# sm-edwards/CrossScale-ECG-A-Modular-HPC-Pipeline-from-Locality-Optimization-to-MPI-GPU-Overlap

Hardware: AMD Instinct MI355X
Metric: ECG samples/sec (node) + conv1d speedup vs torch.Conv1d, tiny 1D-CNN at 1/2/4/8 GPU (higher is better)
Workload: dtype bf16; 1 GPU; model=TinyECG (1458 params), global_batch=256, seq_len=500, parallelism=dp1, sync=fedavg every 50 local steps (none all_reduce AVG, overlap=none), per_client_batch=256, max_windows_per_client=20000, backend=fused

## Files before the change

csrc/kernels/tiny_ecg_step.hip:

```cpp
#include "../include/ecg_common.h"

#include <climits>
#include <cstdint>
#include <cstdlib>
#include <cstring>
#include <type_traits>

namespace {

constexpr int C = 16;
constexpr int K1 = 7;
constexpr int K2 = 5;
constexpr int MAX_CLASSES = 16;
constexpr int MAX_PAIRS_PER_WAVE = 4;

struct Layout {
  int w1, b1, w2, b2, wh, bh, P;
};

__host__ __device__ inline Layout make_layout(int nc) {
  Layout l;
  l.w1 = 0;
  l.b1 = C * K1;
  l.w2 = l.b1 + C;
  l.b2 = l.w2 + C * C * K2;
  l.wh = l.b2 + C;
  l.bh = l.wh + nc * C;
  l.P = l.bh + nc;
  return l;
}

struct Smem {
  int Lp;
  int xs_off, xcol_off, h1_off, dh2_off, ps_off, frag_off, red_off, bytes;
};

constexpr int RED_G = 0;
constexpr int RED_POOLED = 16;
constexpr int RED_POOL = 48;

struct FusedOpt {
  int slab_wt;
};
__host__ __device__ constexpr int msplit(int waves) { return (waves - 1) / 5 < 1 ? 1 : (waves - 1) / 5; }
__host__ __device__ constexpr int red_cnt(int waves) { return RED_POOL + waves * 16; }
__host__ __device__ constexpr int red_m(int waves) { return red_cnt(waves) + waves * 16; }
__host__ __device__ constexpr int red_dw1(int waves) { return red_m(waves) + msplit(waves) * 1280; }
__host__ __device__ constexpr int red_head(int waves) { return red_dw1(waves) + waves * 128; }
__host__ __device__ constexpr int red_floats(int waves) { return red_head(waves) + 288; }

__device__ __forceinline__ __amdgpu_buffer_rsrc_t make_rsrc(const void* p, long bytes) {
  return __builtin_amdgcn_make_buffer_rsrc(const_cast<void*>(p), (short)0, (int)bytes, 0x00020000);
}
__device__ __forceinline__ void st_wt(__amdgpu_buffer_rsrc_t r, int idx, float v) {
  __builtin_amdgcn_raw_buffer_store_b32(__builtin_bit_cast(unsigned, v), r, idx * 4, 0, 16);
}
__device__ __forceinline__ void st_wt4(__amdgpu_buffer_rsrc_t r, int idx, f32x4 v) {
  typedef int i32x4 __attribute__((ext_vector_type(4)));
  __builtin_amdgcn_raw_buffer_store_b128(__builtin_bit_cast(i32x4, v), r, idx * 4, 0, 16);
}
__device__ __forceinline__ float ld_wt(__amdgpu_buffer_rsrc_t r, int idx) {
  return __builtin_bit_cast(float, __builtin_amdgcn_raw_buffer_load_b32(r, idx * 4, 0, 16));
}

constexpr int F32_KSTEPS = C * K2 / 4;

constexpr int WP_FRAGF = 0;
constexpr int WP_FRAGD = 3 * 64 * 8;
constexpr int WP_AW1 = 2 * 3 * 64 * 8;
constexpr int WP_B2_BYTE = (WP_AW1 + C * 8) * 2;
constexpr int WP_BYTES = WP_B2_BYTE + C * 4;
constexpr int kParamsW2End = C * K1 + C + C * C * K2;

__host__ __device__ constexpr int frag_bias_elem(int co) { return (2 * 64 + 32 + co) * 8; }
__host__ __device__ constexpr bool frag_pad_is_bias(int which, int l, int j) { return which == 0 && j == 0 && l < 48; }

__device__ __forceinline__ void wprep_put(unsigned char* wp, int i, float v) {
  __bf16* wb = reinterpret_cast<__bf16*>(wp);
  if (i < C * K1) {
    wb[WP_AW1 + (i / K1) * 8 + i % K1] = ecg::to_bf16(v);
  } else if (i < C * K1 + C) {
    wb[WP_AW1 + (i - C * K1) * 8 + 7] = ecg::to_bf16(v);
  } else if (i < kParamsW2End) {
    const int e = i - (C * K1 + C);
    const int co = e / (C * K2), ci = (e / K2) % C, k = e % K2;
    const int rf = 16 * k + ci, rd = 16 * k + co;
    const __bf16 bv = ecg::to_bf16(v);
    wb[WP_FRAGF + ((rf >> 5) * 64 + 16 * ((rf & 31) >> 3) + co) * 8 + (rf & 7)] = bv;
    wb[WP_FRAGD + ((rd >> 5) * 64 + 16 * ((rd & 31) >> 3) + ci) * 8 + (rd & 7)] = bv;
  } else if (i < kParamsW2End + C) {
    reinterpret_cast<float*>(wp + WP_B2_BYTE)[i - kParamsW2End] = v;
    wb[WP_FRAGF + frag_bias_elem(i - kParamsW2End)] = ecg::to_bf16(v);
  }
}

__global__ __launch_bounds__(256) void tiny_prep_kernel(const float* __restrict__ params,
                                                        unsigned char* __restrict__ wp,
                                                        const int* __restrict__ idx_src, int* __restrict__ idx_dst,
                                                        long n_idx) {
  const int tid = threadIdx.x;
  if (blockIdx.x == 0) {
    for (int i = tid; i < kParamsW2End + C; i += 256) wprep_put(wp, i, params[i]);
    __bf16* wb = reinterpret_cast<__bf16*>(wp);
    for (int e = tid; e < 2 * 32 * 8; e += 256) {
      const int which = e >> 8, l = 32 + ((e >> 3) & 31), j = e & 7;
      if (!frag_pad_is_bias(which, l, j)) wb[(which ? WP_FRAGD : WP_FRAGF) + (2 * 64 + l) * 8 + j] = ecg::to_bf16(0.f);
    }
    return;
  }
  const long base = (long)(blockIdx.x - 1) * 1024;
  for (long i = base + tid; i < n_idx && i < base + 1024; i += 256) idx_dst[i] = idx_src[i];
}

__host__ __device__ inline Smem make_smem(int L, int waves, int nc = MAX_CLASSES, bool f32 = false) {
  Smem s;
  s.Lp = (L + 31) / 32 * 32;
  s.xs_off = 0;
  s.xcol_off = s.xs_off + ((s.Lp + 16) * 4 + 15) / 16 * 16;
  s.h1_off = s.xcol_off + (f32 ? 0 : (s.Lp + 1) * 16);
  const int act_bytes = (s.Lp + 8) * C * (f32 ? 4 : 2);
  s.dh2_off = s.h1_off + act_bytes;
  s.ps_off = s.dh2_off + act_bytes;
  const int ps_bytes = ((make_layout(nc).P) * 4 + 15) / 16 * 16;
  s.frag_off = s.ps_off + ps_bytes;
  s.red_off = s.frag_off + (f32 ? 2 * F32_KSTEPS * 64 * 4 : 2 * 3 * 64 * 16);
  s.bytes = s.red_off + (red_floats(waves) * 4 + 15) / 16 * 16;
  return s;
}

__device__ __forceinline__ bf16x8 cat44(s16x4 a, s16x4 b) {
  typedef short s16x8 __attribute__((ext_vector_type(8)));
  s16x8 r;
  r[0] = a[0]; r[1] = a[1]; r[2] = a[2]; r[3] = a[3];
  r[4] = b[0]; r[5] = b[1]; r[6] = b[2]; r[7] = b[3];
  return __builtin_bit_cast(bf16x8, r);
}

__device__ __forceinline__ s16x4 lds_tr16(const __bf16* p) {
  return __builtin_amdgcn_ds_read_tr16_b64_v4i16((__attribute__((address_space(3))) s16x4*)(p));
}

__device__ __forceinline__ float lane_bcast(float v, int src) {
  return __builtin_bit_cast(float, __builtin_amdgcn_readlane(__builtin_bit_cast(int, v), src));
}

__device__ __forceinline__ float row16_sum(float v) {
  v += __builtin_bit_cast(float, __builtin_amdgcn_update_dpp(0, __builtin_bit_cast(int, v), 0x111, 0xf, 0xf, true));
  v += __builtin_bit_cast(float, __builtin_amdgcn_update_dpp(0, __builtin_bit_cast(int, v), 0x112, 0xf, 0xf, true));
  v += __builtin_bit_cast(float, __builtin_amdgcn_update_dpp(0, __builtin_bit_cast(int, v), 0x114, 0xf, 0xf, true));
  v += __builtin_bit_cast(float, __builtin_amdgcn_update_dpp(0, __builtin_bit_cast(int, v), 0x118, 0xf, 0xf, true));
  return v;
}

template <int WAVES, bool F32, bool PF = false>
struct TinySample {
  static_assert(!(PF && F32), "prepared fragments are bf16 operands");
  using AT = std::conditional_t<F32, float, __bf16>;
  static constexpr int NT = WAVES * 64;
  Smem sm;
  Layout lay;
  int L, Lp, NP, nc;
  int tid, lane, w, h, c;
  float* xs;
  __bf16* xcol;
  AT* h1s;
  AT* ms;
  float* ps;
  __bf16* fragF;
  __bf16* fragD;
  float* fragF32;
  float* fragD32;
  float* red;
  uint32_t mask1 = 0u;
  bf16x8 pf_aw, pf_wf[3], pf_wd[3];

  __device__ __forceinline__ void pf_load_fwd(const unsigned char* __restrict__ wp) {
    const __bf16* wb = reinterpret_cast<const __bf16*>(wp);
    if (h == 0) {
      pf_aw = *reinterpret_cast<const bf16x8*>(wb + WP_AW1 + c * 8);
    } else {
#pragma unroll
      for (int j = 0; j < 8; ++j) pf_aw[j] = ecg::to_bf16(0.f);
    }
#pragma unroll
    for (int s = 0; s < 3; ++s) pf_wf[s] = *reinterpret_cast<const bf16x8*>(wb + WP_FRAGF + (s * 64 + lane) * 8);
  }
  __device__ __forceinline__ void pf_load_dgrad(const unsigned char* __restrict__ wp) {
    const __bf16* wb = reinterpret_cast<const __bf16*>(wp);
    if (w == 0) {
#pragma unroll
      for (int s = 0; s < 3; ++s) pf_wd[s] = *reinterpret_cast<const bf16x8*>(wb + WP_FRAGD + (s * 64 + lane) * 8);
    }
  }

  __device__ __forceinline__ TinySample(unsigned char* smem, int L_, int nc_)
      : sm(make_smem(L_, WAVES, nc_, F32)), lay(make_layout(nc_)), L(L_), nc(nc_) {
    Lp = sm.Lp;
    NP = Lp / 32;
    xs = reinterpret_cast<float*>(smem + sm.xs_off);
    xcol = reinterpret_cast<__bf16*>(smem + sm.xcol_off);
    h1s = reinterpret_cast<AT*>(smem + sm.h1_off);
    ms = reinterpret_cast<AT*>(smem + sm.dh2_off);
    ps = reinterpret_cast<float*>(smem + sm.ps_off);
    fragF = reinterpret_cast<__bf16*>(smem + sm.frag_off);
    fragD = fragF + 3 * 64 * 8;
    fragF32 = reinterpret_cast<float*>(smem + sm.frag_off);
    fragD32 = fragF32 + F32_KSTEPS * 64;
    red = reinterpret_cast<float*>(smem + sm.red_off);
    tid = threadIdx.x;
    lane = tid & 63;
    w = __builtin_amdgcn_readfirstlane(tid >> 6);
    h = lane >> 4;
    c = lane & 15;
  }

  static constexpr int XK = (32 * MAX_PAIRS_PER_WAVE * WAVES + 16 + NT - 1) / NT;
  struct XRegs {
    float v[XK];
  };
  __device__ __forceinline__ void load_x(const float* __restrict__ xrow, XRegs& r) const {
#pragma unroll
    for (int k = 0; k < XK; ++k) {
      const int i = tid + k * NT, t = i - 3;
      if (k * NT < Lp + 16) {
        const float v = xrow[min(max(t, 0), L - 1)];
        r.v[k] = (i < Lp + 16 && t >= 0 && t < L) ? v : 0.f;
      }
    }
  }
  __device__ __forceinline__ void put_x(const XRegs& r) {
#pragma unroll
    for (int k = 0; k < XK; ++k) {
      const int i = tid + k * NT;
      if (i < Lp + 16) xs[i] = r.v[k];
    }
  }
  __device__ __forceinline__ void stage_x(const float* __restrict__ xrow) {
    XRegs r;
    load_x(xrow, r);
    put_x(r);
  }

  __device__ __forceinline__ void put_param(int i, float v) {
    ps[i] = v;
    if constexpr (!F32) {
      if (i >= lay.b2 && i < lay.b2 + C) fragF[frag_bias_elem(i - lay.b2)] = ecg::to_bf16(v);
    }
    const int e = i - lay.w2;
    if (e >= 0 && e < C * C * K2) {
      const int co = e / (C * K2), ci = (e / K2) % C, k = e % K2;
      const int rf = 16 * k + ci, rd = 16 * k + co;
      if constexpr (F32) {
        fragF32[(rf >> 2) * 64 + 16 * (rf & 3) + co] = v;
        fragD32[(rd >> 2) * 64 + 16 * (rd & 3) + ci] = v;
      } else {
        const __bf16 bv = ecg::to_bf16(v);
        fragF[((rf >> 5) * 64 + 16 * ((rf & 31) >> 3) + co) * 8 + (rf & 7)] = bv;
        fragD[((rd >> 5) * 64 + 16 * ((rd & 31) >> 3) + ci) * 8 + (rd & 7)] = bv;
      }
    }
  }

  __device__ __forceinline__ void zero_pads() {
    if constexpr (!F32) {
      for (int e = PF ? 2 * 32 * 8 : tid; e < 2 * 32 * 8; e += NT) {
        const int which = e >> 8, l = 32 + ((e >> 3) & 31), j = e & 7;
        if (!frag_pad_is_bias(which, l, j)) (which ? fragD : fragF)[(2 * 64 + l) * 8 + j] = ecg::to_bf16(0.f);
      }
      if (tid < 4) reinterpret_cast<uint32_t*>(xcol + Lp * 8)[tid] = 0u;
    }
    constexpr int DW = C * (int)sizeof(AT) / 4;
    uint32_t* h1w = reinterpret_cast<uint32_t*>(h1s);
    uint32_t* mw = reinterpret_cast<uint32_t*>(ms);
    for (int i = tid; i < 8 * DW; i += NT) {
      const int r = i / DW, d = i % DW;
      const int hr = r < 2 ? r : Lp + 2 + (r - 2);
      h1w[hr * DW + d] = 0u;
      const int dr = r < 4 ? r : Lp + 4 + (r - 4);
      mw[dr * DW + d] = 0u;
    }
  }

  __device__ __forceinline__ void conv1() {
    if constexpr (!F32) {
      bf16x8 Aw;
      if constexpr (PF) {
        Aw = pf_aw;
      } else {
#pragma unroll
        for (int j = 0; j < 8; ++j) {
          const float v = j < K1 ? ps[lay.w1 + c * K1 + j] : ps[lay.b1 + c];
          Aw[j] = ecg::to_bf16(h == 0 ? v : 0.f);
        }
      }
      const __bf16* xb = xcol + (h == 0 ? (lane & 15) * 8 : Lp * 8);
      const int tstride = h == 0 ? 16 * 8 : 0;
      const int ntiles = Lp / 16;
      const int j0 = 2 * h;
#pragma unroll 1
      for (int pi = 0; pi < 2 * MAX_PAIRS_PER_WAVE; pi += 2) {
        if (w + pi * WAVES >= ntiles) break;
        int tile[2];
        float v0[2], v1[2];
#pragma unroll
        for (int u = 0; u < 2; ++u) {
          tile[u] = min(w + (pi + u) * WAVES, ntiles - 1);
          const int t = 16 * tile[u] + (lane & 15);
          v0[u] = xs[t + j0];
          v1[u] = j0 + 1 < K1 ? xs[t + j0 + 1] : 1.f;
        }
        const bool has2 = w + (pi + 1) * WAVES < ntiles;
#pragma unroll
        for (int u = 0; u < 2; ++u) {
          const int t = 16 * tile[u] + (lane & 15);
          const bool tv = t < L;
          bf16x2 pr;
          pr[0] = ecg::to_bf16(tv ? v0[u] : 0.f);
          pr[1] = ecg::to_bf16(tv ? v1[u] : 0.f);
          *reinterpret_cast<bf16x2*>(xcol + t * 8 + j0) = pr;
        }
        bf16x8 Bx[2];
#pragma unroll
        for (int u = 0; u < 2; ++u) Bx[u] = *reinterpret_cast<const bf16x8*>(xb + tile[u] * tstride);
#pragma unroll
        for (int u = 0; u < 2; ++u) {
          if (u == 1 && !has2) break;
          const f32x4 acc = __builtin_amdgcn_mfma_f32_16x16x32_bf16(Aw, Bx[u], f32x4{0.f, 0.f, 0.f, 0.f}, 0, 0, 0);
          bf16x4 o;
#pragma unroll
          for (int i = 0; i < 4; ++i) o[i] = (AT)fmaxf(acc[i], 0.f);
          *reinterpret_cast<bf16x4*>(h1s + (16 * tile[u] + (lane & 15) + 2) * C + 4 * h) = o;
        }
      }
      return;
    }
    mask1 = 0u;
    float w1r[K1];
#pragma unroll
    for (int k = 0; k < K1; ++k) w1r[k] = ps[lay.w1 + c * K1 + k];
    const float b1r = ps[lay.b1 + c];
#pragma unroll
    for (int pi = 0; pi < MAX_PAIRS_PER_WAVE; ++pi) {
      const int pair = w + pi * WAVES;
      if (pair < NP) {
#pragma unroll
        for (int half = 0; half < 2; ++half) {
          const int t0 = 32 * pair + 16 * half + 4 * h;
          float xw[12];
#pragma unroll
          for (int q4 = 0; q4 < 3; ++q4) {
            const float4 v = reinterpret_cast<const float4*>(xs + t0)[q4];
            xw[4 * q4] = v.x; xw[4 * q4 + 1] = v.y; xw[4 * q4 + 2] = v.z; xw[4 * q4 + 3] = v.w;
          }
#pragma unroll
          for (int i = 0; i < 4; ++i) {
            const int t = t0 + i;
            float v = b1r;
#pragma unroll
            for (int k = 0; k < K1; ++k) v = fmaf(w1r[k], xw[i + k], v);
            v = (t < L) ? fmaxf(v, 0.f) : 0.f;
            const AT vb = (AT)v;
            h1s[(t + 2) * C + c] = vb;
            mask1 |= ((float)vb > 0.f ? 1u : 0u) << (pi * 8 + half * 4 + i);
          }
        }
      }
    }
  }

  __device__ __forceinline__ void conv2() {
    if constexpr (!F32) {
      bf16x8 Wf[3];
      float pool[4];
      if constexpr (PF) {
#pragma unroll
        for (int s = 0; s < 3; ++s) Wf[s] = pf_wf[s];
      } else {
#pragma unroll
        for (int s = 0; s < 3; ++s) Wf[s] = *reinterpret_cast<const bf16x8*>(fragF + (s * 64 + lane) * 8);
      }
      bf16x8 Bone;
#pragma unroll
      for (int j = 0; j < 8; ++j) Bone[j] = ecg::to_bf16(0.f);
      if (h == 2) Bone[0] = ecg::to_bf16(1.f);
#pragma unroll
      for (int i = 0; i < 4; ++i) pool[i] = 0.f;
#pragma unroll
      for (int pi = 0; pi < MAX_PAIRS_PER_WAVE; ++pi) {
        const int pair = w + pi * WAVES;
        if (pair < NP) {
          bf16x8 Bh[2][3];
#pragma unroll
          for (int half = 0; half < 2; ++half)
#pragma unroll
            for (int s = 0; s < 3; ++s) {
              const int r = 32 * pair + 16 * half + (lane & 15) + 2 * s + (h >> 1) - 2;
              if (s == 2 && h >= 2)
                Bh[half][s] = Bone;
              else
                Bh[half][s] = *reinterpret_cast<const bf16x8*>(h1s + (r + 2) * C + 8 * (h & 1));
            }
          f32x4 accs[2];
#pragma unroll
          for (int half = 0; half < 2; ++half) {
            accs[half] = f32x4{0.f, 0.f, 0.f, 0.f};
#pragma unroll
            for (int s = 0; s < 3; ++s)
              accs[half] = __builtin_amdgcn_mfma_f32_16x16x32_bf16(Wf[s], Bh[half][s], accs[half], 0, 0, 0);
          }
          auto epilogue = [&](auto masked) {
#pragma unroll
            for (int half = 0; half < 2; ++half) {
              const int t = 32 * pair + 16 * half + (lane & 15);
              const bool tv = !decltype(masked)::value || t < L;
              bf16x4 mk;
#pragma unroll
              for (int i = 0; i < 4; ++i) {
                const float a = tv ? accs[half][i] : 0.f;
                pool[i] += fmaxf(a, 0.f);
                mk[i] = ecg::to_bf16(__builtin_amdgcn_fmed3f(a * 0x1p126f, 0.f, 1.f));
              }
              *reinterpret_cast<bf16x4*>(ms + (t + 4) * C + 4 * h) = mk;
            }
          };
          if (32 * pair + 32 <= L)
            epilogue(std::false_type{});
          else
            epilogue(std::true_type{});
        }
      }
#pragma unroll
      for (int i = 0; i < 4; ++i) pool[i] = row16_sum(pool[i]);
      if ((lane & 15) == 15) {
#pragma unroll
        for (int i = 0; i < 4; ++i) red[RED_POOL + w * 16 + 4 * h + i] = pool[i];
      }
      return;
    }
    bf16x8 Bf[3];
    float Wf[F32_KSTEPS];
    if constexpr (F32) {
#pragma unroll
      for (int s = 0; s < F32_KSTEPS; ++s) Wf[s] = fragF32[s * 64 + lane];
    } else {
#pragma unroll
      for (int s = 0; s < 3; ++s) Bf[s] = *reinterpret_cast<const bf16x8*>(fragF + (s * 64 + lane) * 8);
    }
    const float b2r = ps[lay.b2 + c];
    float pool = 0.f, cnt = 0.f;
#pragma unroll
    for (int pi = 0; pi < MAX_PAIRS_PER_WAVE; ++pi) {
      const int pair = w + pi * WAVES;
      if (pair < NP) {
#pragma unroll
        for (int half = 0; half < 2; ++half) {
          const int t0 = 32 * pair + 16 * half;
          f32x4 acc = {0.f, 0.f, 0.f, 0.f};
          if constexpr (F32) {
#pragma unroll
            for (int s = 0; s < F32_KSTEPS; ++s) {
              const int r = 4 * s + h, tap = r >> 4, ci = r & 15;
              const float a = h1s[(t0 + (lane & 15) + tap - 2 + 2) * C + ci];
              acc = __builtin_amdgcn_mfma_f32_16x16x4f32(a, Wf[s], acc, 0, 0, 0);
            }
          } else {
#pragma unroll
            for (int s = 0; s < 3; ++s) {
              const int tap = 2 * s + (h >> 1);
              const int r = t0 + (lane & 15) + tap - 2;
              const bf16x8 A = *reinterpret_cast<const bf16x8*>(h1s + (r + 2) * C + 8 * (h & 1));
              acc = __builtin_amdgcn_mfma_f32_16x16x32_bf16(A, Bf[s], acc, 0, 0, 0);
            }
          }
#pragma unroll
          for (int i = 0; i < 4; ++i) {
            const int t = t0 + 4 * h + i;
            float v = fmaxf(acc[i] + b2r, 0.f);
            if (t >= L) v = 0.f;
            pool += v;
            const bool on = v > 0.f;
            cnt += on ? 1.f : 0.f;
            ms[(t + 4) * C + c] = (AT)(on ? 1.f : 0.f);
          }
        }
      }
    }
    pool = ecg::quarter_sum(pool);
    cnt = ecg::quarter_sum(cnt);
    if (lane < 16) {
      red[RED_POOL + w * 16 + lane] = pool;
      red[red_cnt(WAVES) + w * 16 + lane] = cnt;
    }
  }

  template <bool TRAIN>
  __device__ __forceinline__ void head_and_M(int ylab, float inv_B, float* out, int out_stride, int b) {
    if (w == 0) {
      float pp[WAVES];
#pragma unroll
      for (int ww = 0; ww < WAVES; ++ww) pp[ww] = red[RED_POOL + ww * 16 + c];
      float pooled = 0.f;
#pragma unroll
      for (int ww = 0; ww < WAVES; ++ww) pooled += pp[ww];
      pooled *= 1.0f / (float)L;
      float pv[C];
#pragma unroll
      for (int co = 0; co < C; ++co) pv[co] = lane_bcast(pooled, co);
      const int n = c;
      float logit = -INFINITY;
      if (n < nc) {
        const float4* whr = reinterpret_cast<const float4*>(ps + lay.wh + n * C);
        logit = ps[lay.bh + n];
#pragma unroll
        for (int q4 = 0; q4 < C / 4; ++q4) {
          const float4 wv4 = whr[q4];
          logit = fmaf(wv4.x, pv[4 * q4], logit);
          logit = fmaf(wv4.y, pv[4 * q4 + 1], logit);
          logit = fmaf(wv4.z, pv[4 * q4 + 2], logit);
          logit = fmaf(wv4.w, pv[4 * q4 + 3], logit);
        }
      }
      if constexpr (!TRAIN) {
        if (lane < nc) out[(long)b * out_stride + n] = logit;
      } else {
        float m = -INFINITY;
        for (int nn = 0; nn < nc; ++nn) m = fmaxf(m, lane_bcast(logit, nn));
        const float e = (n < nc) ? __expf(logit - m) : 0.f;
        float ssum = 0.f;
        for (int nn = 0; nn < nc; ++nn) ssum += lane_bcast(e, nn);
        const int y = __builtin_amdgcn_readfirstlane(ylab);
        const float loss = m + __logf(ssum) - lane_bcast(logit, y);
        const float dlogit = (n < nc) ? (e / ssum - (n == y ? 1.f : 0.f)) * inv_B : 0.f;
        float* hg = red + red_head(WAVES);
        if (lane < nc) {
          float4* hr = reinterpret_cast<float4*>(hg + n * C);
#pragma unroll
          for (int q4 = 0; q4 < C / 4; ++q4)
            hr[q4] = make_float4(dlogit * pv[4 * q4], dlogit * pv[4 * q4 + 1], dlogit * pv[4 * q4 + 2],
                                 dlogit * pv[4 * q4 + 3]);
          hg[nc * C + n] = dlogit;
        }
        if (lane == 0) hg[nc * C + nc] = loss;
        float dp = 0.f;
        for (int nn = 0; nn < nc; ++nn) dp = fmaf(lane_bcast(dlogit, nn), ps[lay.wh + nn * C + c], dp);
        const float gl = dp * (1.0f / (float)L);
        if (lane < 16) red[RED_G + c] = gl;
        if constexpr (PF) {
          float gq[8];
#pragma unroll
          for (int j = 0; j < 8; ++j) {
            const float lo = lane_bcast(gl, j), hi = lane_bcast(gl, 8 + j);
            gq[j] = (h & 1) ? hi : lo;
          }
#pragma unroll
          for (int s = 0; s < 3; ++s) {
            bf16x8 sc;
#pragma unroll
            for (int j = 0; j < 8; ++j) sc[j] = ecg::to_bf16(ecg::from_bf16(pf_wd[s][j]) * gq[j]);
            *reinterpret_cast<bf16x8*>(fragD + (s * 64 + lane) * 8) = sc;
          }
        }
      }
    } else if (TRAIN && w <= 5 * msplit(WAVES)) {
      constexpr int S = msplit(WAVES);
      const int item = w - 1, k = item / S, part = item % S;
      const int per = (NP + S - 1) / S;
      const int p0 = part * per, p1 = p0 + per < NP ? p0 + per : NP;
      f32x4 acc = {0.f, 0.f, 0.f, 0.f};
      if constexpr (F32) {
        for (int pair = p0; pair < p1; ++pair) {
#pragma unroll
          for (int s = 0; s < 8; ++s) {
            const int t = 32 * pair + 4 * s + h;
            const float a = ms[(t + 4) * C + (lane & 15)];
            const float bb = h1s[(t + k - 2 + 2) * C + (lane & 15)];
            acc = __builtin_amdgcn_mfma_f32_16x16x4f32(a, bb, acc, 0, 0, 0);
          }
        }
      } else {
        const int q = (lane & 15) >> 2, p4 = (lane & 3) * 4;
        bf16x8 ones;
#pragma unroll
        for (int j = 0; j < 8; ++j) ones[j] = ecg::to_bf16(1.f);
        f32x4 cnt1 = {0.f, 0.f, 0.f, 0.f}, cnt2 = {0.f, 0.f, 0.f, 0.f};
        auto mfma_pair = [&](int pair, f32x4 a, f32x4& cn) {
          const int ta = 32 * pair + 4 * h + q;
          const bf16x8 A = cat44(lds_tr16(ms + (ta + 4) * C + p4), lds_tr16(ms + (ta + 16 + 4) * C + p4));
          const bf16x8 Bm =
              cat44(lds_tr16(h1s + (ta + k - 2 + 2) * C + p4), lds_tr16(h1s + (ta + 16 + k - 2 + 2) * C + p4));
          if (k == 2) cn = __builtin_amdgcn_mfma_f32_16x16x32_bf16(A, ones, cn, 0, 0, 0);
          return __builtin_amdgcn_mfma_f32_16x16x32_bf16(A, Bm, a, 0, 0, 0);
        };
        f32x4 acc2 = {0.f, 0.f, 0.f, 0.f};
        int pair = p0;
        for (; pair + 1 < p1; pair += 2) {
          acc = mfma_pair(pair, acc, cnt1);
          acc2 = mfma_pair(pair + 1, acc2, cnt2);
        }
        if (pair < p1) acc = mfma_pair(pair, acc, cnt1);
#pragma unroll
        for (int i = 0; i < 4; ++i) acc[i] += acc2[i];
        if (k == 2 && (lane & 15) == 0) {
#pragma unroll
          for (int i = 0; i < 4; ++i) red[red_cnt(WAVES) + part * 16 + 4 * h + i] = cnt1[i] + cnt2[i];
        }
      }
      float* pm = red + red_m(WAVES) + part * 1280;
#pragma unroll
      for (int i = 0; i < 4; ++i) pm[(4 * h + i) * (C * K2) + c * K2 + k] = acc[i];
    }
  }

  __device__ __forceinline__ void dgrad() {
    float gq[8];
#pragma unroll
    for (int q2 = 0; q2 < 2; ++q2) {
      const float4 v = reinterpret_cast<const float4*>(red + RED_G + 8 * (h & 1))[q2];
      gq[4 * q2] = v.x; gq[4 * q2 + 1] = v.y; gq[4 * q2 + 2] = v.z; gq[4 * q2 + 3] = v.w;
    }
    bf16x8 Bd[3];
    float Wd[F32_KSTEPS];
    if constexpr (!F32) {
      if constexpr (PF) {
#pragma unroll
        for (int s = 0; s < 3; ++s) Bd[s] = *reinterpret_cast<const bf16x8*>(fragD + (s * 64 + lane) * 8);
      } else {
#pragma unroll
        for (int s = 0; s < 3; ++s) {
          const bf16x8 raw = *reinterpret_cast<const bf16x8*>(fragD + (s * 64 + lane) * 8);
#pragma unroll
          for (int j = 0; j < 8; ++j) Bd[s][j] = ecg::to_bf16(ecg::from_bf16(raw[j]) * gq[j]);
        }
      }
      const int q = (lane & 15) >> 2, p4 = (lane & 3) * 4;
      const __bf16* xzero = xcol + Lp * 8;
      f32x4 wacc = {0.f, 0.f, 0.f, 0.f};
#pragma unroll
      for (int pi = 0; pi < MAX_PAIRS_PER_WAVE; ++pi) {
        const int pair = w + pi * WAVES;
        if (pair < NP) {
          bf16x8 Am[2][3];
          bf16x4 hv[2];
          const __bf16* mbase = ms + (32 * pair + (lane & 15) - (h >> 1) + 2) * C + 8 * (h & 1);
#pragma unroll
          for (int half = 0; half < 2; ++half) {
            const int t0 = 32 * pair + 16 * half;
#pragma unroll
            for (int s = 0; s < 3; ++s)
              Am[half][s] = *reinterpret_cast<const bf16x8*>(mbase + (16 * half + 4 - 2 * s) * C);
            hv[half] = *reinterpret_cast<const bf16x4*>(h1s + (t0 + (lane & 15) + 2) * C + 4 * h);
          }
          f32x4 accs[2];
#pragma unroll
          for (int half = 0; half < 2; ++half) {
            accs[half] = f32x4{0.f, 0.f, 0.f, 0.f};
#pragma unroll
            for (int s = 0; s < 3; ++s)
              accs[half] = __builtin_amdgcn_mfma_f32_16x16x32_bf16(Bd[s], Am[half][s], accs[half], 0, 0, 0);
          }
#pragma unroll
          for (int half = 0; half < 2; ++half) {
            const int t0 = 32 * pair + 16 * half;
            typedef unsigned u32x2 __attribute__((ext_vector_type(2)));
            const u32x2 hb = __builtin_bit_cast(u32x2, hv[half]);
            u32x2 db;
#pragma unroll
            for (int q2 = 0; q2 < 2; ++q2) {
              const unsigned nz = (hb[q2] & 0x7fff7fffu) + 0x7fff7fffu;
              typedef short s16x2 __attribute__((ext_vector_type(2)));
              const s16x2 m = __builtin_bit_cast(s16x2, nz) >> (short)15;
              bf16x2 pr;
              pr[0] = ecg::to_bf16(accs[half][2 * q2]);
              pr[1] = ecg::to_bf16(accs[half][2 * q2 + 1]);
              db[q2] = __builtin_bit_cast(unsigned, pr) & __builtin_bit_cast(unsigned, m);
            }
            *reinterpret_cast<u32x2*>(h1s + (t0 + (lane & 15) + 2) * C + 4 * h) = db;
          }
          const int ta = 32 * pair + 4 * h + q;
          const bf16x8 Ad = cat44(lds_tr16(h1s + (ta + 2) * C + p4), lds_tr16(h1s + (ta + 16 + 2) * C + p4));
          const __bf16* xa = p4 < 8 ? xcol + ta * 8 + p4 : xzero;
          const __bf16* xb = p4 < 8 ? xcol + (ta + 16) * 8 + p4 : xzero;
          wacc = __builtin_amdgcn_mfma_f32_16x16x32_bf16(Ad, cat44(lds_tr16(xa), lds_tr16(xb)), wacc, 0, 0, 0);
        }
      }
      if ((lane & 15) < 8) {
#pragma unroll
        for (int i = 0; i < 4; ++i) red[red_dw1(WAVES) + w * 128 + (4 * h + i) * 8 + (lane & 15)] = wacc[i];
      }
      return;
    }
    if constexpr (F32) {
#pragma unroll
      for (int s = 0; s < F32_KSTEPS; ++s) Wd[s] = fragD32[s * 64 + lane] * red[RED_G + ((4 * s + h) & 15)];
    } else {
#pragma unroll
      for (int s = 0; s < 3; ++s) {
        const bf16x8 raw = *reinterpret_cast<const bf16x8*>(fragD + (s * 64 + lane) * 8);
#pragma unroll
        for (int j = 0; j < 8; ++j) Bd[s][j] = ecg::to_bf16(ecg::from_bf16(raw[j]) * gq[j]);
      }
    }
    float dw1[K1 + 1];
#pragma unroll
    for (int k = 0; k <= K1; ++k) dw1[k] = 0.f;
#pragma unroll
    for (int pi = 0; pi < MAX_PAIRS_PER_WAVE; ++pi) {
      const int pair = w + pi * WAVES;
      if (pair < NP) {
#pragma unroll
        for (int half = 0; half < 2; ++half) {
          const int t0 = 32 * pair + 16 * half;
          f32x4 acc = {0.f, 0.f, 0.f, 0.f};
          if constexpr (F32) {
#pragma unroll
            for (int s = 0; s < F32_KSTEPS; ++s) {
              const int r = 4 * s + h, k = r >> 4, co = r & 15;
              const float a = ms[(t0 + (lane & 15) - k + 2 + 4) * C + co];
              acc = __builtin_amdgcn_mfma_f32_16x16x4f32(a, Wd[s], acc, 0, 0, 0);
            }
          } else {
#pragma unroll
            for (int s = 0; s < 3; ++s) {
              const int k = 2 * s + (h >> 1);
              const int r = t0 + (lane & 15) - k + 2;
              const bf16x8 A = *reinterpret_cast<const bf16x8*>(ms + (r + 4) * C + 8 * (h & 1));
              acc = __builtin_amdgcn_mfma_f32_16x16x32_bf16(A, Bd[s], acc, 0, 0, 0);
            }
          }
          const int tb = t0 + 4 * h;
          float xw[12];
#pragma unroll
          for (int q4 = 0; q4 < 3; ++q4) {
            const float4 v = reinterpret_cast<const float4*>(xs + tb)[q4];
            xw[4 * q4] = v.x; xw[4 * q4 + 1] = v.y; xw[4 * q4 + 2] = v.z; xw[4 * q4 + 3] = v.w;
          }
#pragma unroll
          for (int i = 0; i < 4; ++i) {
            const bool on = (mask1 >> (pi * 8 + half * 4 + i)) & 1u;
            const float d = on ? acc[i] : 0.f;
            dw1[K1] += d;
#pragma unroll
            for (int k = 0; k < K1; ++k) dw1[k] = fmaf(d, xw[i + k], dw1[k]);
          }
        }
      }
    }
#pragma unroll
    for (int k = 0; k <= K1; ++k) {
      const float v = ecg::quarter_sum(dw1[k]);
      if (lane < 16) red[red_dw1(WAVES) + w * 128 + c * 8 + k] = v;
    }
  }

  __device__ __forceinline__ float row_value(int i) const {
    float v = 0.f;
    if (i >= lay.wh) {
      v = red[red_head(WAVES) + (i - lay.wh)];
    } else if (i < lay.b1) {
      const int o = red_dw1(WAVES) + (i / K1) * 8 + (i % K1);
#pragma unroll
      for (int ww = 0; ww < WAVES; ++ww) v += red[o + ww * 128];
    } else if (i < lay.w2) {
      const int o = red_dw1(WAVES) + (i - lay.b1) * 8 + K1;
#pragma unroll
      for (int ww = 0; ww < WAVES; ++ww) v += red[o + ww * 128];
    } else if (i < lay.b2) {
      const int e = i - lay.w2;
#pragma unroll
      for (int part = 0; part < msplit(WAVES); ++part) v += red[red_m(WAVES) + part * 1280 + e];
      v *= red[RED_G + e / (C * K2)];
    } else {
      const int co = i - lay.b2;
      constexpr int NCP = F32 ? WAVES : msplit(WAVES);
#pragma unroll
      for (int pp = 0; pp < NCP; ++pp) v += red[red_cnt(WAVES) + pp * 16 + co];
      v *= red[RED_G + co];
    }
    return v;
  }

  __device__ __forceinline__ void row_store(__amdgpu_buffer_rsrc_t r, int rowbase) const {
    constexpr int NQ = C * C * K2 / 4;
    static_assert(NQ + 128 + C <= NT || WAVES < 16, "one job per thread at 16 waves");
    if (tid < NQ) {
      const int e0 = 4 * tid;
      f32x4 v = *reinterpret_cast<const f32x4*>(red + red_m(WAVES) + e0);
#pragma unroll
      for (int part = 1; part < msplit(WAVES); ++part) {
        const f32x4 u = *reinterpret_cast<const f32x4*>(red + red_m(WAVES) + part * 1280 + e0);
        v[0] += u[0]; v[1] += u[1]; v[2] += u[2]; v[3] += u[3];
      }
      const float g = red[RED_G + e0 / (C * K2)];
#pragma unroll
      for (int q = 0; q < 4; ++q) v[q] *= g;
      st_wt4(r, rowbase + lay.w2 + e0, v);
    } else {
      const int i = tid < NQ + 128 ? tid - NQ : lay.b2 + (tid - NQ - 128);
      if (i <= lay.P) st_wt(r, rowbase + i, row_value(i));
    }
  }
};

template <int WAVES, int MODE, bool F32, bool PF>
__global__ __launch_bounds__(WAVES * 64) void tiny_ecg_step_kernel(
    const float* __restrict__ X, int L, long ldx,
    const int* __restrict__ idx,
    const int* __restrict__ Y,
    const float* __restrict__ params, int nc,
    float* __restrict__ out, int out_stride,
    float inv_B, unsigned long long* __restrict__ stamps,
    FusedOpt opt, const unsigned char* __restrict__ wprep) {
  extern __shared__ __attribute__((aligned(16))) unsigned char smem[];
  TinySample<WAVES, F32, PF> S(smem, L, nc);
  constexpr bool TRAIN = MODE != 1;
  const int tid = threadIdx.x;
  const int b = blockIdx.x;
  const __amdgpu_buffer_rsrc_t slab_r = make_rsrc(out, (long)gridDim.x * out_stride * 4);
  const int rowbase = b * out_stride;
  if (stamps && tid == 0) stamps[(long)b * 16 + 15] = __builtin_amdgcn_s_memrealtime();
#pragma unroll 1
  for (int rep = 0; rep < (MODE == 2 ? 2 : 1); ++rep) {
#define ECG_STAMP(k) \
  if (stamps && tid == 0) stamps[(long)b * 16 + 7 * rep + (k)] = __builtin_amdgcn_s_memtime();
    ECG_STAMP(0)
    int ylab = 0;
    if constexpr (PF) {
      S.pf_load_fwd(wprep);
      const int i = S.lay.wh + tid;
      const float hv = i < S.lay.P ? params[i] : 0.f;
      {
        const long row = idx ? (long)idx[b] : (long)b;
        if (TRAIN) ylab = Y[row];
        S.stage_x(X + row * ldx);
      }
      if (i < S.lay.P) S.ps[i] = hv;
      static_assert(MAX_CLASSES * C + MAX_CLASSES <= 8 * 64, "head parameters: one per thread");
    } else {
      constexpr int PR = 4;
      float pv[PR];
#pragma unroll
      for (int j = 0; j < PR; ++j) {
        const int i = tid + j * S.NT;
        pv[j] = i < S.lay.P ? params[i] : 0.f;
      }
      {
        const long row = idx ? (long)idx[b] : (long)b;
        if (TRAIN) ylab = Y[row];
        S.stage_x(X + row * ldx);
      }
#pragma unroll
      for (int j = 0; j < PR; ++j) {
        const int i = tid + j * S.NT;
        if (i < S.lay.P) S.put_param(i, pv[j]);
      }
      for (int i = tid + PR * S.NT; i < S.lay.P; i += S.NT) S.put_param(i, params[i]);
    }
    S.zero_pads();
    __syncthreads();
    ECG_STAMP(1)
    S.conv1();
    __syncthreads();
    ECG_STAMP(2)
    S.conv2();
    if constexpr (PF && TRAIN) S.pf_load_dgrad(wprep);
    __syncthreads();
    ECG_STAMP(3)
    S.template head_and_M<TRAIN>(ylab, inv_B, out, out_stride, b);
    if (!TRAIN) return;
    if (MODE == 0 && stamps && (tid & 63) == 0 && (S.w <= 1 || S.w == WAVES - 1))
      stamps[(long)b * 16 + 8 + (S.w == 0 ? 0 : S.w == 1 ? 1 : 2)] = __builtin_amdgcn_s_memtime();
    __syncthreads();
    ECG_STAMP(4)
    S.dgrad();
    __syncthreads();
    ECG_STAMP(5)
    if (WAVES == 16 && opt.slab_wt && S.lay.P - S.lay.b2 + 1 <= S.NT - 448) {
      S.row_store(slab_r, rowbase);
    } else if (opt.slab_wt) {
      for (int i = tid; i <= S.lay.P; i += S.NT) st_wt(slab_r, rowbase + i, S.row_value(i));
    } else {
      for (int i = tid; i <= S.lay.P; i += S.NT) out[rowbase + i] = S.row_value(i);
    }
    ECG_STAMP(6)
#undef ECG_STAMP
    if (MODE == 2) __syncthreads();
  }
  if (stamps && tid == 0) stamps[(long)b * 16 + 14] = __builtin_amdgcn_s_memrealtime();
}

constexpr int kRedColsDefault = 32;
constexpr int RED_ROWG = 16;

struct GatherArgs {
  const float* X;
  long ldx;
  const int* idx;
  const int* Y;
  float* xg;
  int* yg;
  int L, ldg, B, vec;
  int nred;
};
__host__ __device__ inline int gather_rows_per_block(int L, int vec, int nt) {
  const int per_row = vec ? L / 4 : L;
  return per_row >= nt ? 1 : nt / per_row;
}

template <int RED_COLS>
__global__ __launch_bounds__(RED_COLS * RED_ROWG) void slab_reduce_sgd_kernel(
    const float* __restrict__ slab, int G, int stride, int P,
    float* __restrict__ params, float* __restrict__ mom, float* __restrict__ grad_out,
    float* __restrict__ loss_acc, float lr, float momentum, float wd, int nesterov, int apply,
    unsigned char* __restrict__ wprep,
    GatherArgs ga) {
  constexpr int NT = RED_COLS * RED_ROWG;
  if ((int)blockIdx.x >= ga.nred) {
    const int per_row = ga.vec ? ga.L / 4 : ga.L;
    const int rpb = gather_rows_per_block(ga.L, ga.vec, NT);
    const int r0 = ((int)blockIdx.x - ga.nred) * rpb;
    const __amdgpu_buffer_rsrc_t xr = make_rsrc(ga.xg, (long)ga.B * ga.ldg * 4);
    for (int e = threadIdx.x; e < rpb * per_row; e += NT) {
      const int lr_ = e / per_row, j = e - lr_ * per_row, b = r0 + lr_;
      if (b >= ga.B) break;
      const long row = ga.idx[b];
      if (ga.vec) {
        st_wt4(xr, b * ga.ldg + 4 * j, *reinterpret_cast<const f32x4*>(ga.X + row * ga.ldx + 4 * j));
      } else {
        st_wt(xr, b * ga.ldg + j, ga.X[row * ga.ldx + j]);
      }
      if (j == 0) ga.yg[b] = ga.Y[row];
    }
    return;
  }
  __shared__ float part[RED_ROWG][RED_COLS + 1];
  const int cl = threadIdx.x % RED_COLS, rg = threadIdx.x / RED_COLS;
  const int col = blockIdx.x * RED_COLS + cl;
  const bool upd = rg == 0 && col < P && apply;
  const float p0 = upd ? params[col] : 0.f;
  const float m0 = (upd && momentum != 0.f) ? mom[col] : 0.f;
  float s = 0.f;
  if (col <= P) {
    const float* base = slab + col;
    int r = rg;
    for (; r + RED_ROWG * 15 < G; r += RED_ROWG * 16) {
      float v[16];
#pragma unroll
      for (int j = 0; j < 16; ++j) v[j] = base[(long)(r + RED_ROWG * j) * stride];
#pragma unroll
      for (int j = 0; j < 16; j += 2) s += v[j] + v[j + 1];
    }
    for (; r < G; r += RED_ROWG) s += base[(long)r * stride];
  }
  part[rg][cl] = s;
  __syncthreads();
  if (rg == 0 && col <= P) {
    float gsum = 0.f;
#pragma unroll
    for (int j = 0; j < RED_ROWG; ++j) gsum += part[j][cl];
    if (col == P) {
      if (loss_acc) loss_acc[0] += gsum;
    } else {
      if (grad_out) grad_out[col] = gsum;
      if (apply) {
        const float p = p0;
        float d = gsum + wd * p;
        if (momentum != 0.f) {
          const float bm = momentum * m0 + d;
          mom[col] = bm;
          d = nesterov ? d + momentum * bm : bm;
        }
        const float pn = p - lr * d;
        params[col] = pn;
        if (wprep) wprep_put(wprep, col, pn);
      }
    }
  }
}

unsigned long long* g_stamps = nullptr;


template <int WAVES, int MODE, bool F32, bool PF>
int launch_step(const float* X, int L, long ldx, const int* idx, const int* Y, const float* params, int nc,
                float* out, int out_stride, int B, float inv_B, const FusedOpt& opt, const unsigned char* wprep,
                hipStream_t stream) {
  const Smem sm = make_smem(L, WAVES, nc, F32);
  auto kern = tiny_ecg_step_kernel<WAVES, MODE, F32, PF>;
  if (sm.bytes > 64 * 1024)
    ECG_HIP_CHECK(hipFuncSetAttribute((const void*)kern, hipFuncAttributeMaxDynamicSharedMemorySize, sm.bytes));
  hipLaunchKernelGGL(kern, dim3(B), dim3(WAVES * 64), sm.bytes, stream, X, L, ldx, idx, Y, params, nc, out,
                     out_stride, inv_B, g_stamps, opt, wprep);
  ECG_HIP_CHECK(hipGetLastError());
  return ecg::kOk;
}

int launch_prep(const float* params, unsigned char* wprep, const int* idx_src, int* idx_dst, long n_idx,
                hipStream_t stream) {
  if (!params || !wprep || (n_idx > 0 && (!idx_src || !idx_dst))) return ecg::kBadArg;
  const long nb = 1 + (n_idx > 0 ? (n_idx + 1023) / 1024 : 0);
  hipLaunchKernelGGL(tiny_prep_kernel, dim3((unsigned)nb), dim3(256), 0, stream, params, wprep, idx_src, idx_dst,
                     n_idx > 0 ? n_idx : 0);
  ECG_HIP_CHECK(hipGetLastError());
  return ecg::kOk;
}

constexpr int kMaxLds = 160 * 1024;

int g_forced_waves = 0;
int pick_waves(int L, bool f32) {
  const int Lp = (L + 31) / 32 * 32;
  const int forced = g_forced_waves;
  const bool fit16 = Lp <= 32 * 4 * 16 && make_smem(L, 16, MAX_CLASSES, f32).bytes <= kMaxLds;
  if (forced == 16 && fit16) return 16;
  if (forced == 8) return 8;
  return (fit16 && Lp / 32 >= 16) ? 16 : 8;
}

int check_step_args(int L, int nc, int B, int out_stride, int mode, bool f32 = false) {
  if (L < 8 || B <= 0 || nc < 1 || nc > MAX_CLASSES) return ecg::kBadArg;
  const int Lp = (L + 31) / 32 * 32;
  if (Lp > 32 * 4 * 8 || make_smem(L, 8, MAX_CLASSES, f32).bytes > kMaxLds) return ecg::kTooLarge;
  const Layout lay = make_layout(nc);
  if (mode != 1 && out_stride < lay.P + 1) return ecg::kBadArg;
  if (mode == 1 && out_stride < nc) return ecg::kBadArg;
  return ecg::kOk;
}

template <bool F32, bool PF>
int dispatch_cfg(int mode, int waves, const float* X, int L, long ldx, const int* idx, const int* Y,
                 const float* params, int nc, float* out, int out_stride, int B, float inv_B, const FusedOpt& opt,
                 const unsigned char* wprep, hipStream_t stream) {
  if (mode == 2)
    return launch_step<8, 2, F32, PF>(X, L, ldx, idx, Y, params, nc, out, out_stride, B, inv_B, opt, wprep, stream);
  if (mode == 0)
    return waves == 8
               ? launch_step<8, 0, F32, PF>(X, L, ldx, idx, Y, params, nc, out, out_stride, B, inv_B, opt, wprep, stream)
               : launch_step<16, 0, F32, PF>(X, L, ldx, idx, Y, params, nc, out, out_stride, B, inv_B, opt, wprep,
                                             stream);
  return waves == 8
             ? launch_step<8, 1, F32, PF>(X, L, ldx, idx, Y, params, nc, out, out_stride, B, inv_B, opt, wprep, stream)
             : launch_step<16, 1, F32, PF>(X, L, ldx, idx, Y, params, nc, out, out_stride, B, inv_B, opt, wprep, stream);
}

int step_dispatch(int mode, int prec, const float* X, int L, long ldx, const int* idx, const int* Y,
                  const float* params, int nc, float* out, int out_stride, int B, float inv_B, const FusedOpt& opt,
                  const unsigned char* wprep, hipStream_t stream) {
  if (prec != 0 && prec != 1) return ecg::kBadArg;
  int st = check_step_args(L, nc, B, out_stride, mode, prec == 1);
  if (st) return st;
  if (wprep && prec == 1) return ecg::kBadArg;
  const int waves = pick_waves(L, prec == 1);
  if (prec == 1)
    return dispatch_cfg<true, false>(mode, waves, X, L, ldx, idx, Y, params, nc, out, out_stride, B, inv_B, opt,
                                     nullptr, stream);
  if (wprep)
    return dispatch_cfg<false, true>(mode, waves, X, L, ldx, idx, Y, params, nc, out, out_stride, B, inv_B, opt,
                                     wprep, stream);
  return dispatch_cfg<false, false>(mode, waves, X, L, ldx, idx, Y, params, nc, out, out_stride, B, inv_B, opt,
                                    nullptr, stream);
}

FusedOpt no_fuse() {
  FusedOpt o{};
  o.slab_wt = 1;
  return o;
}

int reduce_dispatch(const float* slab, int G, int stride, int P, float* params, float* mom, float* grad_out,
                    float* loss_acc, float lr, float momentum, float wd, int nesterov, int apply,
                    unsigned char* wprep, hipStream_t stream, const GatherArgs* gather = nullptr) {
  if (G <= 0 || P <= 0 || stride < P + 1) return ecg::kBadArg;
  if (apply && (!params || (momentum != 0.f && !mom))) return ecg::kBadArg;
  constexpr int cols = kRedColsDefault;
  const int blocks = (P + 1 + cols - 1) / cols;
  GatherArgs ga{};
  ga.nred = INT_MAX;
  int grid = blocks;
  if (gather) {
    ga = *gather;
    ga.nred = blocks;
    const int rpb = gather_rows_per_block(ga.L, ga.vec, cols * RED_ROWG);
    grid += (ga.B + rpb - 1) / rpb;
  }
  hipLaunchKernelGGL(slab_reduce_sgd_kernel<cols>, dim3(grid), dim3(cols * RED_ROWG), 0, stream, slab, G, stride, P,
                     params, mom, grad_out, loss_acc, lr, momentum, wd, nesterov, apply, wprep, ga);
  ECG_HIP_CHECK(hipGetLastError());
  return ecg::kOk;
}

struct RoundGraph {
  hipGraph_t graph = nullptr;
  hipGraphExec_t exec = nullptr;
  int steps = 0;
};

}

ECG_API int ecg_tiny_param_count(int nc) { return make_layout(nc).P; }

ECG_API int ecg_tiny_set_stamps(unsigned long long* stamps) {
  g_stamps = stamps;
  return ecg::kOk;
}

ECG_API int ecg_tiny_force_waves(int waves) {
  pick_waves(32, false);
  const int prev = g_forced_waves;
  g_forced_waves = (waves == 8 || waves == 16) ? waves : 0;
  return prev;
}

ECG_API int ecg_tiny_smem_bytes(int L, int prec) {
  return make_smem(L, pick_waves(L, prec == 1), MAX_CLASSES, prec == 1).bytes;
}

ECG_API int ecg_tiny_wprep_bytes(void) { return WP_BYTES; }

ECG_API int ecg_tiny_prep(const float* params, void* wprep, hipStream_t stream) {
  return launch_prep(params, static_cast<unsigned char*>(wprep), nullptr, nullptr, 0, stream);
}

static int prep_then(int mode, int prec, const float* X, int L, long ldx, const int* idx, const int* Y,
                     const float* params, int nc, float* out, int out_stride, int B, float inv_B, void* wprep,
                     hipStream_t stream) {
  if (wprep) {
    if (prec != 0) return ecg::kBadArg;
    const int st = launch_prep(params, static_cast<unsigned char*>(wprep), nullptr, nullptr, 0, stream);
    if (st) return st;
  }
  return step_dispatch(mode, prec, X, L, ldx, idx, Y, params, nc, out, out_stride, B, inv_B, no_fuse(),
                       static_cast<const unsigned char*>(wprep), stream);
}

ECG_API int ecg_tiny_step_grads(const float* X, int L, long ldx, const int* idx, const int* Y,
                                const float* params, int nc, float* slab, int slab_stride, int B, float inv_B,
                                int prec, void* wprep, hipStream_t stream) {
  return prep_then(0, prec, X, L, ldx, idx, Y, params, nc, slab, slab_stride, B, inv_B, wprep, stream);
}

ECG_API int ecg_tiny_step_grads_twice(const float* X, int L, long ldx, const int* idx, const int* Y,
                                      const float* params, int nc, float* slab, int slab_stride, int B, float inv_B,
                                      int prec, void* wprep, hipStream_t stream) {
  return prep_then(2, prec, X, L, ldx, idx, Y, params, nc, slab, slab_stride, B, inv_B, wprep, stream);
}

ECG_API int ecg_tiny_forward(const float* X, int L, long ldx, const int* idx, const float* params, int nc,
                             float* logits, int B, int prec, void* wprep, hipStream_t stream) {
  return prep_then(1, prec, X, L, ldx, idx, nullptr, params, nc, logits, nc, B, 0.f, wprep, stream);
}

ECG_API int ecg_slab_reduce_sgd(const float* slab, int G, int stride, int P, float* params, float* mom,
                                float* grad_out, float* loss_acc, float lr, float momentum, float wd, int nesterov,
                                int apply, void* wprep, hipStream_t stream) {
  if (wprep && !apply) return ecg::kBadArg;
  return reduce_dispatch(slab, G, stride, P, params, mom, grad_out, loss_acc, lr, momentum, wd, nesterov, apply,
                         static_cast<unsigned char*>(wprep), stream);
}

static int train_step(const float* X, int L, long ldx, const int* idx, const int* Y, float* params, float* mom,
                      int nc, float* slab, int slab_stride, int B, float* loss_acc, float lr, float momentum, float wd,
                      int nesterov, int prec, unsigned char* wprep, int image, hipStream_t stream,
                      const GatherArgs* gather = nullptr) {
  int st = ecg::kOk;
// ... 148 lines not shown
```

Baseline: 24.83 million samples/s.

## Load conv1 input windows directly from global into registers, skip x staging

For bf16 kernels, the input row is no longer staged into shared memory. Each lane now loads its 7-tap window straight from global memory with bounded buffer loads and builds the im2col MFMA operand in registers. The first tile's loads are issued early, alongside parameter loading, and the barrier before conv1 is dropped; the xs shared region is also removed from the layout. This trades one shared-memory pass and a sync for redundant global loads of overlapping windows and more register pressure.

```diff
diff --git a/csrc/kernels/tiny_ecg_step.hip b/csrc/kernels/tiny_ecg_step.hip
--- a/csrc/kernels/tiny_ecg_step.hip
+++ b/csrc/kernels/tiny_ecg_step.hip
@@ -62,6 +62,10 @@
 __device__ __forceinline__ float ld_wt(__amdgpu_buffer_rsrc_t r, int idx) {
   return __builtin_bit_cast(float, __builtin_amdgcn_raw_buffer_load_b32(r, idx * 4, 0, 16));
 }
+__device__ __forceinline__ float ld_bounded(__amdgpu_buffer_rsrc_t r, int byte_off) {
+  return __builtin_bit_cast(float, __builtin_amdgcn_raw_buffer_load_b32(r, byte_off, 0, 0));
+}
+constexpr int kOobByte = 0x40000000;
 
 constexpr int F32_KSTEPS = C * K2 / 4;
 
@@ -116,7 +120,7 @@
   Smem s;
   s.Lp = (L + 31) / 32 * 32;
   s.xs_off = 0;
-  s.xcol_off = s.xs_off + ((s.Lp + 16) * 4 + 15) / 16 * 16;
+  s.xcol_off = s.xs_off + (f32 ? ((s.Lp + 16) * 4 + 15) / 16 * 16 : 0);
   s.h1_off = s.xcol_off + (f32 ? 0 : (s.Lp + 1) * 16);
   const int act_bytes = (s.Lp + 8) * C * (f32 ? 4 : 2);
   s.dh2_off = s.h1_off + act_bytes;
@@ -174,6 +178,14 @@
   uint32_t mask1 = 0u;
   bf16x8 pf_aw, pf_wf[3], pf_wd[3];
 
+  __device__ __forceinline__ void load_aw(const float* __restrict__ params) {
+#pragma unroll
+    for (int j = 0; j < 8; ++j) {
+      const float v = j < K1 ? params[lay.w1 + c * K1 + j] : params[lay.b1 + c];
+      pf_aw[j] = ecg::to_bf16(h == 0 ? v : 0.f);
+    }
+  }
+
   __device__ __forceinline__ void pf_load_fwd(const unsigned char* __restrict__ wp) {
     const __bf16* wb = reinterpret_cast<const __bf16*>(wp);
     if (h == 0) {
@@ -241,6 +253,39 @@
     put_x(r);
   }
 
+  struct X1 {
+    float v[2][K1];
+  };
+  __device__ __forceinline__ int conv1_t(int pi, int u) const {
+    return 16 * min(w + (pi + u) * WAVES, Lp / 16 - 1) + (lane & 15);
+  }
+  __device__ __forceinline__ void conv1_load(__amdgpu_buffer_rsrc_t xr, int pi, X1& r) const {
+#pragma unroll
+    for (int u = 0; u < 2; ++u) {
+      const int t = conv1_t(pi, u);
+      const int base = (h == 0 && t < L) ? 4 * max(t - 3, 0) : kOobByte;
+#pragma unroll
+      for (int j = 0; j < K1; ++j) r.v[u][j] = ld_bounded(xr, base + 4 * j);
+    }
+  }
+  __device__ __forceinline__ bf16x8 conv1_operand(const float (&ld)[K1], int t) const {
+    float v[K1];
+#pragma unroll
+    for (int j = 0; j < K1; ++j) v[j] = ld[j];
+    if (h == 0 && t < 3) {
+      const int s = 3 - t;
+#pragma unroll
+      for (int j = K1 - 1; j >= 0; --j) v[j] = (s & 1) ? (j >= 1 ? v[j - 1] : 0.f) : v[j];
+#pragma unroll
+      for (int j = K1 - 1; j >= 0; --j) v[j] = (s & 2) ? (j >= 2 ? v[j - 2] : 0.f) : v[j];
+    }
+    bf16x8 Bx;
+#pragma unroll
+    for (int j = 0; j < K1; ++j) Bx[j] = ecg::to_bf16(v[j]);
+    Bx[7] = ecg::to_bf16(h == 0 && t < L ? 1.f : 0.f);
+    return Bx;
+  }
+
   __device__ __forceinline__ void put_param(int i, float v) {
     ps[i] = v;
     if constexpr (!F32) {
@@ -281,59 +326,40 @@
     }
   }
 
+  __device__ __forceinline__ void conv1_pair(int pi, const X1& x) {
+    const bool has2 = w + (pi + 1) * WAVES < Lp / 16;
+    bf16x8 Bx[2];
+    int t[2];
+#pragma unroll
+    for (int u = 0; u < 2; ++u) {
+      t[u] = conv1_t(pi, u);
+      Bx[u] = conv1_operand(x.v[u], t[u]);
+      if (h == 0) *reinterpret_cast<bf16x8*>(xcol + t[u] * 8) = Bx[u];
+    }
+#pragma unroll
+    for (int u = 0; u < 2; ++u) {
+      if (u == 1 && !has2) break;
+      const f32x4 acc = __builtin_amdgcn_mfma_f32_16x16x32_bf16(pf_aw, Bx[u], f32x4{0.f, 0.f, 0.f, 0.f}, 0, 0, 0);
+      bf16x4 o;
+#pragma unroll
+      for (int i = 0; i < 4; ++i) o[i] = (AT)fmaxf(acc[i], 0.f);
+      *reinterpret_cast<bf16x4*>(h1s + (t[u] + 2) * C + 4 * h) = o;
+    }
+  }
+  __device__ __forceinline__ void conv1_mfma(__amdgpu_buffer_rsrc_t xr, const X1& x0) {
+    const int ntiles = Lp / 16;
+    if (w < ntiles) conv1_pair(0, x0);
+#pragma unroll 1
+    for (int pi = 2; pi < 2 * MAX_PAIRS_PER_WAVE; pi += 2) {
+      if (w + pi * WAVES >= ntiles) break;
+      X1 x;
+      conv1_load(xr, pi, x);
+      conv1_pair(pi, x);
+    }
+  }
+
   __device__ __forceinline__ void conv1() {
-    if constexpr (!F32) {
-      bf16x8 Aw;
-      if constexpr (PF) {
-        Aw = pf_aw;
-      } else {
-#pragma unroll
-        for (int j = 0; j < 8; ++j) {
-          const float v = j < K1 ? ps[lay.w1 + c * K1 + j] : ps[lay.b1 + c];
-          Aw[j] = ecg::to_bf16(h == 0 ? v : 0.f);
-        }
-      }
-      const __bf16* xb = xcol + (h == 0 ? (lane & 15) * 8 : Lp * 8);
-      const int tstride = h == 0 ? 16 * 8 : 0;
-      const int ntiles = Lp / 16;
-      const int j0 = 2 * h;
-#pragma unroll 1
-      for (int pi = 0; pi < 2 * MAX_PAIRS_PER_WAVE; pi += 2) {
-        if (w + pi * WAVES >= ntiles) break;
-        int tile[2];
-        float v0[2], v1[2];
-#pragma unroll
-        for (int u = 0; u < 2; ++u) {
-          tile[u] = min(w + (pi + u) * WAVES, ntiles - 1);
-          const int t = 16 * tile[u] + (lane & 15);
-          v0[u] = xs[t + j0];
-          v1[u] = j0 + 1 < K1 ? xs[t + j0 + 1] : 1.f;
-        }
-        const bool has2 = w + (pi + 1) * WAVES < ntiles;
-#pragma unroll
-        for (int u = 0; u < 2; ++u) {
-          const int t = 16 * tile[u] + (lane & 15);
-          const bool tv = t < L;
-          bf16x2 pr;
-          pr[0] = ecg::to_bf16(tv ? v0[u] : 0.f);
-          pr[1] = ecg::to_bf16(tv ? v1[u] : 0.f);
-          *reinterpret_cast<bf16x2*>(xcol + t * 8 + j0) = pr;
-        }
-        bf16x8 Bx[2];
-#pragma unroll
-        for (int u = 0; u < 2; ++u) Bx[u] = *reinterpret_cast<const bf16x8*>(xb + tile[u] * tstride);
-#pragma unroll
-        for (int u = 0; u < 2; ++u) {
-          if (u == 1 && !has2) break;
-          const f32x4 acc = __builtin_amdgcn_mfma_f32_16x16x32_bf16(Aw, Bx[u], f32x4{0.f, 0.f, 0.f, 0.f}, 0, 0, 0);
-          bf16x4 o;
-#pragma unroll
-          for (int i = 0; i < 4; ++i) o[i] = (AT)fmaxf(acc[i], 0.f);
-          *reinterpret_cast<bf16x4*>(h1s + (16 * tile[u] + (lane & 15) + 2) * C + 4 * h) = o;
-        }
-      }
-      return;
-    }
+    static_assert(F32, "bf16 kernels run conv1_mfma");
     mask1 = 0u;
     float w1r[K1];
 #pragma unroll
@@ -824,15 +850,16 @@
   if (stamps && tid == 0) stamps[(long)b * 16 + 7 * rep + (k)] = __builtin_amdgcn_s_memtime();
     ECG_STAMP(0)
     int ylab = 0;
+    const long row = idx ? (long)idx[b] : (long)b;
+    const float* xrow = X + row * ldx;
+    [[maybe_unused]] const __amdgpu_buffer_rsrc_t xr = make_rsrc(xrow, (long)L * 4);
+    [[maybe_unused]] typename TinySample<WAVES, F32, PF>::X1 x0;
     if constexpr (PF) {
       S.pf_load_fwd(wprep);
       const int i = S.lay.wh + tid;
       const float hv = i < S.lay.P ? params[i] : 0.f;
-      {
-        const long row = idx ? (long)idx[b] : (long)b;
-        if (TRAIN) ylab = Y[row];
-        S.stage_x(X + row * ldx);
-      }
+      if (TRAIN) ylab = Y[row];
+      S.conv1_load(xr, 0, x0);
       if (i < S.lay.P) S.ps[i] = hv;
       static_assert(MAX_CLASSES * C + MAX_CLASSES <= 8 * 64, "head parameters: one per thread");
     } else {
@@ -843,10 +870,12 @@
         const int i = tid + j * S.NT;
         pv[j] = i < S.lay.P ? params[i] : 0.f;
       }
-      {
-        const long row = idx ? (long)idx[b] : (long)b;
-        if (TRAIN) ylab = Y[row];
-        S.stage_x(X + row * ldx);
+      if constexpr (!F32) S.load_aw(params);
+      if (TRAIN) ylab = Y[row];
+      if constexpr (F32) {
+        S.stage_x(xrow);
+      } else {
+        S.conv1_load(xr, 0, x0);
       }
 #pragma unroll
       for (int j = 0; j < PR; ++j) {
@@ -856,9 +885,14 @@
       for (int i = tid + PR * S.NT; i < S.lay.P; i += S.NT) S.put_param(i, params[i]);
     }
     S.zero_pads();
-    __syncthreads();
-    ECG_STAMP(1)
-    S.conv1();
+    if constexpr (F32) {
+      __syncthreads();
+      ECG_STAMP(1)
+      S.conv1();
+    } else {
+      ECG_STAMP(1)
+      S.conv1_mfma(xr, x0);
+    }
     __syncthreads();
     ECG_STAMP(2)
     S.conv2();
```

Result: faster. 25.42 million samples/s, median of 6 (+2.3%).
